# NVIDIA/tensorrt-laboratory

Measured on NVIDIA H100. Metric: ResNet-50 fp16 b=8 inferences/sec, higher is better.
Workload: dtype f16

## Files before the change

### tensorrt_laboratory_b200/csrc/engine.cu

```cuda
#include <cuda.h>
#include <cuda_runtime.h>
#include <stdarg.h>
#include <stdio.h>
#include <stdlib.h>
#include <string.h>

#include <algorithm>
#include <map>
#include <memory>
#include <mutex>
#include <string>
#include <vector>

#include "../../include/b200infer.h"
#include "kernels.h"
#include "plan_format.h"

#include "b2_internal.h"

namespace b2i {
thread_local std::string g_err;
int fail(int code, const char* fmt, ...) {
    char buf[1024];
    va_list ap;
// ... 620 lines not shown
        if (t.last_use < t.def) t.last_use = t.def;
        const size_t size = align_up(t.item_bytes * e->max_batch, 1024);
        const int slack = e->half() ? env_int("B2_ARENA_SLACK", env_int("B2_NET", 0) ? 2 : 0) : 0;
        live.erase(std::remove_if(live.begin(), live.end(), [&](const Live& l) { return l.last + slack < t.def; }), live.end());
        std::sort(live.begin(), live.end(), [](const Live& a, const Live& b) { return a.off < b.off; });
        size_t off = 0;
        for (const Live& l : live) {
            if (off + size <= l.off) break;
            off = std::max(off, l.off + l.size);
        }
        t.offset = off;
        live.push_back({off, size, t.last_use});
        top = std::max(top, off + size);
    }
    e->act_bytes = align_up(std::max<size_t>(top, 1024), 1024);
    e->arena_bytes = e->act_bytes + (e->half() ? kSplitWorkspaceBytes : 0);
}

int make_map_2d(CUtensorMap* map, const void* base, uint64_t inner, uint64_t outer, uint32_t box_inner,
                uint32_t box_outer, CUtensorMapSwizzle swz, bool int8 = false) {
    cuuint64_t dims[2] = {inner, outer};
    cuuint64_t strides[1] = {inner * (int8 ? 1u : 2u)};
    cuuint32_t box[2] = {box_inner, box_outer};
    cuuint32_t estr[2] = {1, 1};
    CUresult r = g_encode_tiled(map, int8 ? CU_TENSOR_MAP_DATA_TYPE_UINT8 : CU_TENSOR_MAP_DATA_TYPE_FLOAT16, 2, const_cast<void*>(base), dims, strides, box,
                                estr, CU_TENSOR_MAP_INTERLEAVE_NONE, swz, CU_TENSOR_MAP_L2_PROMOTION_L2_256B,
                                CU_TENSOR_MAP_FLOAT_OOB_FILL_NONE);
    if (r != CUDA_SUCCESS)
        return fail(B2_ECUDA, "cuTensorMapEncodeTiled failed (%d) dims=%llu,%llu box=%u,%u", int(r),
                    (unsigned long long)inner, (unsigned long long)outer, box_inner, box_outer);
    return B2_OK;
}

int make_map_nhwc(CUtensorMap* map, const void* base, int C, int W, int H, int N, uint32_t box_w, uint32_t box_h) {
    cuuint64_t dims[4] = {cuuint64_t(C), cuuint64_t(W), cuuint64_t(H), cuuint64_t(N)};
    cuuint64_t strides[3] = {cuuint64_t(C) * 2, cuuint64_t(C) * 2 * W, cuuint64_t(C) * 2 * W * H};
    cuuint32_t box[4] = {64, box_w, box_h, 1};
    cuuint32_t estr[4] = {1, 1, 1, 1};
    CUresult r = g_encode_tiled(map, CU_TENSOR_MAP_DATA_TYPE_FLOAT16, 4, const_cast<void*>(base), dims, strides, box, estr,
                                CU_TENSOR_MAP_INTERLEAVE_NONE, CU_TENSOR_MAP_SWIZZLE_128B, CU_TENSOR_MAP_L2_PROMOTION_L2_256B,
                                CU_TENSOR_MAP_FLOAT_OOB_FILL_NONE);
    if (r != CUDA_SUCCESS)
        return fail(B2_ECUDA, "cuTensorMapEncodeTiled(4-D) failed (%d) C=%d W=%d H=%d N=%d box=%u,%u", int(r), C, W, H, N, box_w, box_h);
    return B2_OK;
}

int make_map_im2col(CUtensorMap* map, const void* base, int C, int W, int H, int N, uint64_t pix_bytes,
                    uint64_t row_bytes, uint64_t img_bytes, int kh, int kw, int stride_h, int stride_w, int pad_h,
                    int pad_w_lo, int pad_w_hi, uint32_t channels_per_pixel, uint32_t pixels_per_column,
                    CUtensorMapSwizzle swz, bool int8 = false) {
    cuuint64_t dims[4] = {cuuint64_t(C), cuuint64_t(W), cuuint64_t(H), cuuint64_t(N)};
    cuuint64_t strides[3] = {pix_bytes, row_bytes, img_bytes};
    int lower[2] = {-pad_w_lo, -pad_h};
    int upper[2] = {pad_w_hi - (kw - 1), pad_h - (kh - 1)};
    cuuint32_t estr[4] = {1, cuuint32_t(stride_w), cuuint32_t(stride_h), 1};
    CUresult r = g_encode_im2col(map, int8 ? CU_TENSOR_MAP_DATA_TYPE_UINT8 : CU_TENSOR_MAP_DATA_TYPE_FLOAT16, 4, const_cast<void*>(base), dims, strides, lower,
                                 upper, channels_per_pixel, pixels_per_column, estr, CU_TENSOR_MAP_INTERLEAVE_NONE, swz,
                                 CU_TENSOR_MAP_L2_PROMOTION_L2_256B, CU_TENSOR_MAP_FLOAT_OOB_FILL_NONE);
    if (r != CUDA_SUCCESS)
        return fail(B2_ECUDA, "cuTensorMapEncodeIm2col failed (%d) C=%d W=%d H=%d N=%d k=%dx%d s=%dx%d p=%d,%d/%d", int(r), C,
                    W, H, N, kh, kw, stride_h, stride_w, pad_h, pad_w_lo, pad_w_hi);
    if (g_driver_version <= 13010 && img_bytes * uint64_t(N) < 131072)
        reinterpret_cast<uint64_t*>(map)[1] &= ~(1ull << 21);
    return B2_OK;
}

static int g_sms = 132;

ConvConfig pick_conv_config(int M, int cout_phys, int kblocks, int kb, bool residual, const b2_context* c, bool honor_forced,
                            int group_span = 0) {
    const int m_tiles = (M + 127) / 128;
    ConvConfig best{0, 0, 1, 1e30};
    const int bns[4] = {256, 128, 64, 32};
// ... 8 lines not shown
                               size_t(tiles) * splits * 128 * bn * 4 > kSplitWorkspaceBytes))
                continue;
            const int kpc = (kblocks + splits - 1) / splits;
            if (splits > 1 && (splits - 1) * kpc >= kblocks) continue;
            for (int st : stgs) {
                if (!b2k::conv_config_exists(bn, kb, st)) continue;
                if (b2k::conv_smem_bytes(bn, st, residual) > kSmemLimit) continue;
                if (honor_forced && c->force_stages && st != c->force_stages) continue;
                if (!(honor_forced && c->force_stages) && !stage_depth_useful(bn, kb, st, kpc)) continue;
                const double smem = b2k::conv_smem_bytes(bn, st, residual);
                int per_sm = int(double(kSmemLimit) / smem);
                per_sm = std::min(per_sm, bn <= 64 ? 2 : 1);
                per_sm = std::max(1, std::min(per_sm, 8));
                const int ctas = tiles * splits;
                const int waves = (ctas + g_sms * per_sm - 1) / (g_sms * per_sm);
                const int sharing = std::max(1, std::min(per_sm, (ctas + g_sms - 1) / g_sms));
                const double stage_bytes = 16384.0 + bn * 128.0;
                const double t_kb = std::max(stage_bytes / (70000.0 / sharing), 1.0 / st);
                double t_epi = 0.6 + bn / 64.0 * 0.4 + (residual ? 0.4 : 0.0);
                if (splits > 1) t_epi += 1.0 + 0.3 * splits;
                const double t_cta = 2.0 + kpc * t_kb + t_epi;
                double total = waves * t_cta;
                const double traffic = double(ctas) * kpc * stage_bytes;
                total = std::max(total, traffic / 5.0e6 + 2.0);
                if (total < best.est_us) best = ConvConfig{bn, st, splits, total};
            }
        }
    }
    return best;
}

bool conv_is_row_folded(const b2_context* c, const Op& op) {
    const b2plan::OpRec& r = op.r;
    return !c->no_fold && r.cin_phys == 8 && op.kw() * 8 * 2 == 64 && op.sw() == 1 && op.pw_lo() == 0 && op.pw_hi() == 0;
}
int conv_kb(const b2_context* c, const Op& op) {
    if (op.r.cin_phys % 64 == 0) return 64;
    return conv_is_row_folded(c, op) ? 32 : 8;
}
int conv_num_kblocks(const b2_context* c, const Op& op) {
    const b2plan::OpRec& r = op.r;
    if (op.group_span()) return int(r.taps) * (op.group_span() / 64);
    if (r.cin_phys % 64 == 0) return int(r.taps) * (int(r.cin_phys) / 64);
    if (conv_is_row_folded(c, op)) return (op.kh() + 1) / 2;
    return (int(r.taps_phys) + 7) / 8;
}

int conv_halo_rows(const b2_context* c, const Op& op) {
    const b2plan::OpRec& r = op.r;
    const Tensor& ti = c->e->tensors[r.in];
    const Tensor& to = c->e->tensors[r.out];
    if (op.groups > 1 || r.cin_phys % 64 || r.cout_phys % 64 || op.kh() != 3 || op.kw() != 3 || op.sh() != 1 || op.sw() != 1 || op.ph() != 1 ||
        op.pw_lo() != 1 || op.pw_hi() != 1 || r.res >= 0 || !(r.relu & 2) || ti.h != to.h || ti.w != to.w)
        return 0;
    const int wp = int(to.w) + 2;
    if (wp > 128) return 0;
    return std::min(128 / wp, int(to.h));
}

bool conv_on_tensor_cores(const b2_engine* e, const Op& op) {
    const b2plan::OpRec& r = op.r;
    const bool kb64 = r.cin_phys % 64 == 0, kb8 = r.cin_phys == 8;
    return e->half() && (kb64 || kb8) && r.cout_phys % 32 == 0 && (kb64 || r.taps_phys % 2 == 0) && (op.groups == 1 || op.group_span() > 0);
}

bool conv_takes_ws(const b2_context* c, const Op& op) {
    return conv_kb(c, op) == 64 && (op.r.relu & 2) && op.groups == 1 && !(op.r.relu & b2plan::kConvGelu);
}

bool tactic_applies(const b2_context* c, const Op& op, int batch, const ConvConfig& cfg) {
    const b2plan::OpRec& r = op.r;
    const Tensor& to = c->e->tensors[r.out];
    const int span = op.group_span(), kb = conv_kb(c, op);
    if (cfg.bn <= 0 || int(r.cout_phys) % cfg.bn || cfg.splits < 1 || cfg.sps < 1 || cfg.ws < 0) return false;
    if (op.groups > 1 && (!span || span % cfg.bn || cfg.splits > 1)) return false;
    if ((op.groups > 1 || (r.relu & b2plan::kConvGelu)) && (cfg.ws || cfg.cn > 1 || cfg.halo)) return false;
    if (cfg.halo) {
        const int R = conv_halo_rows(c, op), cblocks = int(r.cin_phys) / 64;
        return R && cfg.splits == 1 && !cfg.ws && cfg.cn <= 1 && b2k::conv_halo_config_exists(cfg.bn) && cblocks <= 8 &&
               b2k::conv_halo_smem(cfg.bn, int(to.w), R, cblocks) <= kSmemLimit;
    }
    if (cfg.ws)
        return conv_takes_ws(c, op) && cfg.splits == 1 && cfg.cn <= 1 && b2k::conv_ws_config_exists(cfg.bn, cfg.stages, cfg.sps) &&
               b2k::conv_ws_smem(cfg.bn, cfg.stages, cfg.sps, r.res >= 0) <= kSmemLimit;
    if (!b2k::conv_config_exists(cfg.bn, kb, cfg.stages, cfg.sps) || b2k::conv_smem_bytes(cfg.bn, cfg.stages, r.res >= 0, cfg.sps) > kSmemLimit)
        return false;
    const int grid_n = int(r.cout_phys) / cfg.bn;
    if (cfg.cn > 1 && (kb != 64 || grid_n % cfg.cn || !b2k::conv_cluster_config_exists(cfg.bn, cfg.stages, cfg.sps, cfg.cn))) return false;
    if (cfg.splits > 1) {
        const int nkb = conv_num_kblocks(c, op), kpc = (nkb + cfg.splits - 1) / cfg.splits;
        const int tiles = (batch * int(to.h * to.w) + 127) / 128 * grid_n;
        if (kb != 64 || kpc < 4 || (cfg.splits - 1) * kpc >= nkb || tiles > kMaxSplitTiles ||
            size_t(tiles) * cfg.splits * 128 * cfg.bn * 4 > kSplitWorkspaceBytes)
            return false;
    }
    return true;
}

std::vector<ConvConfig> conv_candidates(const b2_context* c, const Op& op, int batch, int fixed_splits) {
    const b2plan::OpRec& r = op.r;
    const int kbsz = conv_kb(c, op), nkb = conv_num_kblocks(c, op);
    const int m_tiles = (batch * int(c->e->tensors[r.out].h * c->e->tensors[r.out].w) + 127) / 128;
    const bool ws_only = c->force_ws > 0 && conv_takes_ws(c, op);
    auto ok = [&](const ConvConfig& t) { return tactic_applies(c, op, batch, t); };
    std::vector<ConvConfig> out;
    for (int bn : {256, 128, 64, 32}) {
        if (int(r.cout_phys) % bn) continue;
        const int tiles = m_tiles * (int(r.cout_phys) / bn);
        for (int ws = 0; ws <= 1; ++ws)
        for (int sp : {1, 2, 4, 8})
        for (int sps = 1; sps <= 2; ++sps)
        for (int st : {1, 2, 4, 8}) {
            if ((fixed_splits > 0 && sp != fixed_splits) || (ws ? c->force_ws < 0 : ws_only)) continue;
            ConvConfig t{bn, st, sp, 0.0, sps, ws ? std::min(tiles, g_sms) : 0, 1};
            if (!ok(t)) continue;
            if (ws) {
                if (sps == 2 && nkb < 4) continue;
// ... 80 lines not shown
    a.residual = r.res >= 0 ? reinterpret_cast<const __half*>(tptr(r.res)) : nullptr;
    a.out = reinterpret_cast<__half*>(tptr(r.out));
    a.M = M;
    a.Cout = int(r.cout_phys);
    a.taps = fold ? op.kh() : int(r.taps);
    a.taps_phys = fold ? op.kh() : int(r.taps_phys);
    a.kw = fold ? 1 : op.kw();
    a.cblocks = span ? span / 64 : kb64 ? int(r.cin_phys) / 64 : 1;
    a.group_span = span;
    a.num_kblocks = nkb;
    a.HoWo = int(to.h * to.w);
    a.Wo = int(to.w);
    a.stride_h = op.sh();
    a.stride_w = op.sw();
    a.pad_h = op.ph();
    a.pad_w = op.pw_lo();
    a.relu = int(r.relu & (b2plan::kConvRelu | b2plan::kConvGelu));
    a.wpacked = (r.relu & 2) ? w : nullptr;
    const bool tiled = r.k == 1 && op.kw() == 1 && r.stride == 1 && op.sw() == 1 && r.pad_ == 0 && op.pw_lo() == 0 &&
                       op.pw_hi() == 0 && kb64 && (!c->force_im2col || gelu);
    a.a_mode = tiled ? b2k::A_TILED : b2k::A_IM2COL;
    if (cfg.halo) {
        const int R = conv_halo_rows(c, op);
        cl.halo = 1;
        cl.ws_ctas = 0, cl.cn = 1, a.cn = 1, a.splits = 1, cl.stages = kHaloStagesTag, cl.sps = 1;
        a.halo_rows = R;
        cl.grid_m = batch * ((int(to.h) + R - 1) / R);
        int rc = make_map_nhwc(&cl.mapA, tptr(r.in), int(r.cin_phys), int(ti.w), int(ti.h), batch, uint32_t(ti.w) + 2, uint32_t(R) + 2);
        if (rc) return rc;
        rc = make_map_nhwc(&cl.mapOut, tptr(r.out), int(r.cout_phys), int(to.w), int(to.h), batch, uint32_t(to.w) + 2, uint32_t(R));
        cl.mapB = cl.mapA, cl.mapRes = cl.mapOut;
        return rc;
    }
    const CUtensorMapSwizzle swz = kb64 ? CU_TENSOR_MAP_SWIZZLE_128B : (fold ? CU_TENSOR_MAP_SWIZZLE_64B : CU_TENSOR_MAP_SWIZZLE_NONE);
    const uint64_t pix = uint64_t(r.cin_phys) * 2, rowb = uint64_t(ti.w) * pix, imgb = uint64_t(ti.h) * rowb;
    int rc;
    if (tiled)
        rc = make_map_2d(&cl.mapA, tptr(r.in), r.cin_phys, uint64_t(M), 64, uint32_t(128 / cl.cn), swz);
    else if (fold)
        rc = make_map_im2col(&cl.mapA, tptr(r.in), int(r.cin_phys) * op.kw(), int(ti.w) - op.kw() + 1, int(ti.h), batch, pix,
                             rowb, imgb, op.kh(), 1, op.sh(), 1, op.ph(), 0, 0, 32, 128, swz);
    else
        rc = make_map_im2col(&cl.mapA, tptr(r.in), int(r.cin_phys), int(ti.w), int(ti.h), batch, pix, rowb, imgb, op.kh(),
                             op.kw(), op.sh(), op.sw(), op.ph(), op.pw_lo(), op.pw_hi(), uint32_t(cl.kb), uint32_t(128 / cl.cn), swz);
    if (rc) return rc;
    if (r.relu & 2)
        cl.mapB = cl.mapA;
    else
        rc = make_map_2d(&cl.mapB, w, uint64_t(r.taps_phys) * r.cin_phys, r.cout_phys, uint32_t(cl.kb), uint32_t(cl.bn), swz);
    if (rc) return rc;
    const uint32_t ow = cl.bn >= 64 ? 64 : 32;
    const CUtensorMapSwizzle oswz = cl.bn >= 64 ? CU_TENSOR_MAP_SWIZZLE_128B : CU_TENSOR_MAP_SWIZZLE_64B;
    rc = make_map_2d(&cl.mapOut, tptr(r.out), r.cout_phys, uint64_t(M), ow, 128, oswz);
    if (rc) return rc;
    if (r.res >= 0) rc = make_map_2d(&cl.mapRes, tptr(r.res), r.cout_phys, uint64_t(M), ow, 128, oswz);
    else cl.mapRes = cl.mapOut;
    return rc;
}

int make_i8_conv_launch(b2_context* c, const Op& op, int batch, int bn, int stages, b2k::I8ConvLaunch* out) {
    b2_engine* e = c->e;
    const b2plan::OpRec& r = op.r;
    const Tensor& ti = e->tensors[r.in];
    const Tensor& to = e->tensors[r.out];
    auto tptr = [&](int idx) -> uint8_t* { return c->scratch + e->tensors[idx].offset; };
    b2k::I8ConvLaunch& cl = *out;
    memset(&cl, 0, sizeof cl);
    const int M = batch * int(to.h) * int(to.w);
    cl.bn = bn, cl.stages = stages;
    cl.grid_m = (M + 127) / 128;
    cl.grid_n = int(r.cout_phys) / bn;
    b2k::I8ConvArgs& a = cl.args;
    a.wpacked = e->d_payload + r.w_off;
    const float* rq = reinterpret_cast<const float*>(e->d_payload + r.b_off);
// ... 1465 lines not shown
        if (L.kind == L_NET) run = L.net.get();
    if (!run) return fail(B2_EINVAL, "the plan has no persistent network kernel");
    if (n_ctas) *n_ctas = run->ctas;
    if (run->ctas > cap_ctas) return fail(B2_EINVAL, "counter buffer too small (%d CTAs)", run->ctas);
    long long* d = nullptr;
    const size_t bytes = size_t(run->ctas) * 64 * sizeof(long long);
    B2_CUDA(cudaMalloc(&d, bytes));
    cudaMemset(d, 0, bytes);
    cudaStream_t s = static_cast<cudaStream_t>(stream_);
    run->args.dbg = d;
    int rc = run_all(c, *plan, bindings, s);
    cudaError_t se = cudaStreamSynchronize(s);
    run->args.dbg = nullptr;
    if (!rc && se == cudaSuccess) cudaMemcpy(out, d, bytes, cudaMemcpyDeviceToHost);
    cudaFree(d);
    if (rc) return rc;
    if (se != cudaSuccess) return fail(B2_ECUDA, "debug launch failed: %s", cudaGetErrorString(se));
    return B2_OK;
}

const char* b2_context_launch_name(b2_context* c, int batch, int i) {
    static thread_local std::string s;
    const Launch* L = get_launch(c, batch, i);
    if (!L) return nullptr;
    static const char* kinds[] = {"input_cast", "conv_tcgen05", "conv_simt", "maxpool", "avgpool", "fc", "softmax", "output_cast", "net_tcgen05", "tail_pool_fc_softmax",
                                  "quantize", "conv_i8_tcgen05", "avgpool_i8", "output_cast_i8", "embed_ln", "layernorm", "attention_f16_wgmma",
                                  "pooler", "output_cast_rows"};
    s = std::string(kinds[L->kind]) + ":" + L->name;
    if (L->kind == L_CONV_TC)
        s += " bn=" + std::to_string(L->conv.bn) + " kb=" + std::to_string(L->conv.kb) +
             " st=" + std::to_string(L->conv.stages) + "x" + std::to_string(L->conv.sps) +
             (L->conv.ws_ctas ? " ws=" + std::to_string(L->conv.ws_ctas) : std::string()) +
             (L->conv.cn > 1 ? " cn=" + std::to_string(L->conv.cn) : std::string()) + (L->conv.halo ? " halo" : "") +
             (L->conv.args.a_mode == b2k::A_TILED ? " tiled" : " im2col") +
             " grid=" + std::to_string(L->conv.grid_n) + "x" + std::to_string(L->conv.grid_m) + "x" +
             std::to_string(L->conv.args.splits) + " kblk=" + std::to_string(L->conv.args.num_kblocks) +
             (L->conv.args.group_span ? " span=" + std::to_string(L->conv.args.group_span) : std::string()) +
             ((L->conv.args.relu & b2plan::kConvGelu) ? " gelu" : "");
    if (L->kind == L_CONV_I8)
        s += " bn=" + std::to_string(L->i8.bn) + " st=" + std::to_string(L->i8.stages) + (L->i8.args.a_mode == b2k::A_TILED ? " tiled" : " im2col") + " grid=" +
             std::to_string(L->i8.grid_n) + "x" + std::to_string(L->i8.grid_m) + " kblk=" + std::to_string(L->i8.args.num_kblocks);
    if (L->kind == L_NET)
        s += " layers=" + std::to_string(L->net->args.n_layers) + " tiles=" + std::to_string(L->net->args.total_tiles) +
             " ctas=" + std::to_string(L->net->ctas) + " stages=" + std::to_string(L->net->args.stages);
    if (L->side_join >= 0) s += " side";
    return s.c_str();
}
double b2_context_launch_flops(b2_context* c, int batch, int i) {
    const Launch* L = get_launch(c, batch, i);
    return L ? L->flops : 0.0;
}
double b2_context_launch_bytes(b2_context* c, int batch, int i) {
    const Launch* L = get_launch(c, batch, i);
    return L ? L->bytes : 0.0;
}

}
```

### tensorrt_laboratory_b200/csrc/kernels.cu

```cuda
#include "kernels.h"

#include <stdio.h>
#include <stdlib.h>
#include <string.h>

#include "ptx_sm90.cuh"
#include "wgmma_sm90.cuh"

namespace b2k {

template <int BN, int STAGES, int SPS = 1>
struct ConvCfg {
    static constexpr int A_SUBBLK = 128 * 64 * 2;
    static constexpr int B_SUBBLK = BN * 64 * 2;
    static constexpr int A_STAGE = SPS * A_SUBBLK;
    static constexpr int B_STAGE = SPS * B_SUBBLK;
    static constexpr int PIPE_BYTES = STAGES * (A_STAGE + B_STAGE);
    static constexpr int TILE_BYTES = 128 * BN * 2;
    static_assert(TILE_BYTES <= PIPE_BYTES, "the output staging tile reuses the pipeline buffers");
};

__host__ __device__ constexpr int conv_smem_layout_bytes(int bn, int stages, bool residual, int sps = 1) {
    return stages * sps * (128 * 64 * 2 + bn * 64 * 2) + (residual ? 128 * bn * 2 : 0) + 256 + bn * 4 + 1024;
}

constexpr int kConvThreads = 384;
constexpr int kConsumerWarps = 8;

struct FragPos {
    int row0, col0;
    __device__ FragPos(int consumer_warp, int lane)
        : row0(64 * (consumer_warp >> 2) + 16 * (consumer_warp & 3) + (lane >> 2)), col0(2 * (lane & 3)) {}
};

template <int BN, int KB, int STAGES, int SPS, int CN = 1, bool DBG = false, int AV = 0, bool GELU = false>
__global__ void __launch_bounds__(kConvThreads, BN <= 64 ? 2 : 1)
conv_f16_tcgen05(const __grid_constant__ CUtensorMap mapA, const __grid_constant__ CUtensorMap mapB,
                 const __grid_constant__ CUtensorMap mapOut, const __grid_constant__ CUtensorMap mapRes,
                 const ConvArgs p) {
    static_assert(SPS == 1 || KB == 64, "multi-sub-block stages exist for the 64-wide K path only");
    using Cfg = ConvCfg<BN, STAGES, SPS>;
    constexpr int TPS = 64 / KB;
    constexpr int A_SUB = 128 * KB * 2;
    constexpr int B_SUB = BN * KB * 2;
    constexpr int OW = BN >= 64 ? 64 : 32;
    constexpr int OROWB = OW * 2;
    constexpr int NBOX = BN / OW;

    extern __shared__ uint8_t smem_raw[];
    uint8_t* smem = smem_raw + ((1024u - (smem_u32(smem_raw) & 1023u)) & 1023u);
    const bool has_res = p.residual != nullptr;
    uint8_t* sA = smem;
    uint8_t* sB = smem + STAGES * Cfg::A_STAGE;
    uint8_t* sOut = smem;
    uint8_t* sRes = smem + Cfg::PIPE_BYTES;
    uint8_t* tail = sRes + (has_res ? Cfg::TILE_BYTES : 0);
    uint64_t* full_bar = reinterpret_cast<uint64_t*>(tail);
    uint64_t* empty_bar = full_bar + STAGES;
    uint64_t* accum_bar = empty_bar + STAGES;
    uint64_t* res_bar = accum_bar + 1;
    uint32_t* last_flag = reinterpret_cast<uint32_t*>(res_bar + 1);
    float* s_bias = reinterpret_cast<float*>(tail + 256);

    const int warp = threadIdx.x >> 5;
    const int lane = threadIdx.x & 31;
    const int n0 = blockIdx.x * BN;
    const int m0 = blockIdx.y * 128;
    long long* dbg = (DBG && p.dbg) ? p.dbg + 16ll * ((blockIdx.z * gridDim.y + blockIdx.y) * gridDim.x + blockIdx.x) : nullptr;
    if (dbg && threadIdx.x == 0) {
        dbg[0] = clock64();
        unsigned long long gt;
        asm volatile("mov.u64 %0, %%globaltimer;" : "=l"(gt));
        dbg[8] = static_cast<long long>(gt);
        unsigned smid;
// ... 183 lines not shown
    float acc[BN / 2];
    if (warp >= 4) {
        const uint32_t wg = static_cast<uint32_t>(cw >> 2);
        auto release_stage = [&](int st) {
            __syncwarp();
            if (lane == 0) {
                if (cn > 1) {
                    for (uint32_t r = 0; r < static_cast<uint32_t>(cn); ++r) mbar_arrive_cluster(&empty_bar[st], r);
                } else {
                    mbar_arrive(&empty_bar[st]);
                }
            }
        };
        long long mw = 0, mi = 0;
        for (int i = 0; i < nk; ++i) {
            const int s = i % STAGES;
            const uint32_t ph = (i / STAGES) & 1;
            long long m0c = 0, m1c = 0;
            if (dbg) m0c = clock64();
            mbar_wait(&full_bar[s], ph);
            if (dbg) m1c = clock64(), mw += m1c - m0c;
            if (dbg && i == 0 && cw == 0 && lane == 0) dbg[3] = clock64();
            const uint32_t a_addr = smem_u32(sA + s * Cfg::A_STAGE);
            const uint32_t b_addr = smem_u32(sB + s * Cfg::B_STAGE);
            if constexpr (KB == 64) {
                auto mma = [&](int t) {
                    const int u = t >> 2, j = t & 3;
                    const uint64_t ad = make_wgmma_desc(a_addr + u * Cfg::A_SUBBLK + wg * 8192 + j * 32, 16, 1024, WG_SW128);
                    const uint64_t bd = make_wgmma_desc(b_addr + u * Cfg::B_SUBBLK + j * 32, 16, 1024, WG_SW128);
                    wgmma_f16<BN>(acc, ad, bd, (i > 0 || t > 0) ? 1u : 0u);
                };
                if (SPS == 1 || subs_in_step(i) == SPS) wgmma_group<4 * SPS>(mma);
                else wgmma_group<4>(mma);
            } else if constexpr (KB == 32) {
                auto mma = [&](int t) {
                    const int st = t >> 1, j = t & 1;
                    const uint64_t ad = make_wgmma_desc(a_addr + st * A_SUB + wg * 4096 + j * 32, 16, 512, WG_SW64);
                    const uint64_t bd = make_wgmma_desc(b_addr + st * B_SUB + j * 32, 16, 512, WG_SW64);
                    wgmma_f16<BN>(acc, ad, bd, (i > 0 || t > 0) ? 1u : 0u);
                };
                if (sub_tiles(kb_begin + i) == TPS) wgmma_group<2 * TPS>(mma);
                else wgmma_group<2>(mma);
            } else {
                auto mma = [&](int j) {
                    const uint64_t ad = make_wgmma_desc(a_addr + 2 * j * A_SUB + wg * 1024, A_SUB, 128, WG_NOSWZ);
                    const uint64_t bd = make_wgmma_desc(b_addr + 2 * j * B_SUB, B_SUB, 128, WG_NOSWZ);
                    wgmma_f16<BN>(acc, ad, bd, (i > 0 || j > 0) ? 1u : 0u);
                };
                wgmma_group_upto<TPS / 2>(sub_tiles(kb_begin + i) / 2, mma);
            }
            if constexpr (STAGES == 1) {
                wgmma_wait<0>();
                release_stage(0);
            } else {
                wgmma_wait<1>();
                if (i > 0) release_stage((i - 1) % STAGES);
            }
            if (dbg) mi += clock64() - m1c;
        }
        if constexpr (STAGES > 1) {
            wgmma_wait<0>();
            if (nk > 0) release_stage((nk - 1) % STAGES);
        }
        if (dbg && cw == 0 && lane == 0) dbg[4] = clock64(), dbg[14] = mw, dbg[15] = mi;
    }

    if (warp == 3 && KB == 64) {
        for (int i = 0; i < nk; ++i) {
            const int s = i % STAGES;
            if (i >= STAGES) mbar_wait(&empty_bar[s], ((i / STAGES) & 1) ^ 1);
            if (elect_one_sync()) load_b(kb_begin + i * SPS, s);
            __syncwarp();
        }
    }

// ... 70 lines not shown
                    for (int sp = 0; sp < p.splits; ++sp) {
                        const float2 t = __ldcg(reinterpret_cast<const float2*>(ws_tile + static_cast<size_t>(sp) * (128 * BN) + row * BN + col));
                        f0 += t.x;
                        f1 += t.y;
                    }
                    finish_pair(row, col, f0, f1);
                }
            }
        }
    }
    if (dbg && threadIdx.x == 128) dbg[6] = clock64();
    if (p.pdl_trigger == 2) pdl_launch_dependents();
    fence_proxy_async();
    __syncthreads();
    if (threadIdx.x == 0 && do_store) {
#pragma unroll
        for (int b = 0; b < NBOX; ++b) tma_store_2d(&mapOut, sOut + b * (128 * OROWB), n0 + b * OW, m0);
        tma_store_commit_and_wait_read();
    }
    if (cn > 1) {
        if (warp == 1) {
            const int first = nk > STAGES ? nk - STAGES : 0;
            for (int i = first; i < nk; ++i) mbar_wait(&empty_bar[i % STAGES], (i / STAGES) & 1);
        }
        __syncthreads();
        cluster_sync_all();
    }
    if (dbg && threadIdx.x == 128) {
        dbg[7] = clock64();
        unsigned long long gt;
        asm volatile("mov.u64 %0, %%globaltimer;" : "=l"(gt));
        dbg[9] = static_cast<long long>(gt);
    }
}

__host__ __device__ constexpr int conv_ws_smem_bytes(int bn, int stages, int sps, bool residual) {
    return stages * sps * (128 * 64 * 2 + bn * 64 * 2) + 2 * 128 * bn * 2 + (residual ? 2 * 128 * bn * 2 : 0) + 256 + 1024;
}

template <int BN, int STAGES, int SPS>
__global__ void __launch_bounds__(kConvThreads, 1)
conv_f16_tcgen05_ws(const __grid_constant__ CUtensorMap mapA, const __grid_constant__ CUtensorMap mapOut,
                    const __grid_constant__ CUtensorMap mapRes, const ConvArgs p) {
    constexpr int A_SUBBLK = 128 * 64 * 2;
    constexpr int B_SUBBLK = BN * 64 * 2;
    constexpr int A_STAGE = SPS * A_SUBBLK;
    constexpr int B_STAGE = SPS * B_SUBBLK;
    constexpr int PIPE_BYTES = STAGES * (A_STAGE + B_STAGE);
    constexpr int TILE_BYTES = 128 * BN * 2;
    constexpr int OW = BN >= 64 ? 64 : 32;
    constexpr int OROWB = OW * 2;
    constexpr int NBOX = BN / OW;

    extern __shared__ uint8_t smem_raw[];
    uint8_t* smem = smem_raw + ((1024u - (smem_u32(smem_raw) & 1023u)) & 1023u);
    const bool has_res = p.residual != nullptr;
    uint8_t* sA = smem;
    uint8_t* sB = smem + STAGES * A_STAGE;
    uint8_t* sOut = smem + PIPE_BYTES;
    uint8_t* sRes = sOut + 2 * TILE_BYTES;
    uint8_t* tail = sRes + (has_res ? 2 * TILE_BYTES : 0);
    uint64_t* full_bar = reinterpret_cast<uint64_t*>(tail);
    uint64_t* empty_bar = full_bar + STAGES;
    uint64_t* res_full = empty_bar + STAGES;
    uint64_t* res_empty = res_full + 2;

// ... 402 lines not shown
        }
    }
    return launch_kernel_cluster(conv_f16_tcgen05<BN, KB, STAGES, SPS, CN>, grid, dim3(kConvThreads), smem, stream, true,
                                 static_cast<unsigned>(CN), L.mapA, L.mapB, L.mapOut, L.mapRes, L.args);
}

template <int BN, int KB, int STAGES, int SPS, int CN = 1>
static int init_one() {
    const int want = conv_smem_layout_bytes(BN, STAGES, true, SPS);
    const int bytes = want > 227 * 1024 ? conv_smem_layout_bytes(BN, STAGES, false, SPS) : want;
    if (CN == 1) {
        int e = static_cast<int>(cudaFuncSetAttribute(conv_f16_tcgen05<BN, KB, STAGES, SPS, 1, true>,
                                                      cudaFuncAttributeMaxDynamicSharedMemorySize, bytes));
        if (e) return e;
        if constexpr (KB == 64) {
            if ((e = static_cast<int>(cudaFuncSetAttribute(conv_f16_tcgen05<BN, KB, STAGES, SPS, 1, false, 1>,
                                                           cudaFuncAttributeMaxDynamicSharedMemorySize, bytes)))) return e;
            if ((e = static_cast<int>(cudaFuncSetAttribute(conv_f16_tcgen05<BN, KB, STAGES, SPS, 1, false, 2>,
                                                           cudaFuncAttributeMaxDynamicSharedMemorySize, bytes)))) return e;
            if ((e = static_cast<int>(cudaFuncSetAttribute(conv_f16_tcgen05<BN, KB, STAGES, SPS, 1, false, 2, true>,
                                                           cudaFuncAttributeMaxDynamicSharedMemorySize, bytes)))) return e;
        }
    }
    return static_cast<int>(cudaFuncSetAttribute(conv_f16_tcgen05<BN, KB, STAGES, SPS, CN>, cudaFuncAttributeMaxDynamicSharedMemorySize, bytes));
}

int conv_smem_bytes(int bn, int stages, bool residual, int sps) { return conv_smem_layout_bytes(bn, stages, residual, sps); }

#define B2_FOR_EACH_CONV(X) \
    X(32, 64, 1, 1) X(32, 64, 2, 1) X(32, 64, 4, 1) X(32, 64, 8, 1) \
    X(64, 64, 1, 1) X(64, 64, 2, 1) X(64, 64, 4, 1) X(64, 64, 8, 1) \
    X(128, 64, 1, 1) X(128, 64, 2, 1) X(128, 64, 4, 1) X(256, 64, 2, 1) X(256, 64, 4, 1) \
    X(32, 64, 2, 2) X(32, 64, 4, 2) X(64, 64, 2, 2) X(64, 64, 4, 2) X(128, 64, 2, 2) X(256, 64, 2, 2) \
    X(32, 8, 2, 1) X(32, 8, 4, 1) X(64, 8, 2, 1) X(64, 8, 4, 1) X(64, 8, 8, 1) X(128, 8, 4, 1) \
    X(32, 32, 2, 1) X(32, 32, 4, 1) X(64, 32, 1, 1) X(64, 32, 2, 1) X(64, 32, 4, 1) X(128, 32, 2, 1) X(128, 32, 4, 1)

int conv_halo_smem(int bn, int w, int r, int cblocks) { return halo_smem_bytes(bn, w, r, cblocks); }
bool conv_halo_config_exists(int bn) { return bn == 64 || bn == 128 || bn == 256; }
static int init_conv_halo_kernels() {
    int e;
    if ((e = static_cast<int>(cudaFuncSetAttribute(conv3x3_halo_tcgen05<64>, cudaFuncAttributeMaxDynamicSharedMemorySize, 227 * 1024)))) return e;
    if ((e = static_cast<int>(cudaFuncSetAttribute(conv3x3_halo_tcgen05<128>, cudaFuncAttributeMaxDynamicSharedMemorySize, 227 * 1024)))) return e;
    if ((e = static_cast<int>(cudaFuncSetAttribute(conv3x3_halo_tcgen05<256>, cudaFuncAttributeMaxDynamicSharedMemorySize, 227 * 1024)))) return e;
    return 0;
}
static int launch_conv_halo(const ConvLaunch& L, cudaStream_t stream) {
    const int R = L.args.halo_rows;
    const size_t smem = size_t(halo_smem_bytes(L.bn, L.args.Wo, R, L.args.cblocks));
    if (smem > 227 * 1024 || R < 1 || R * (L.args.Wo + 2) > 128 || L.args.cblocks > kHaloMaxCBlocks) return static_cast<int>(cudaErrorInvalidValue);
    dim3 grid(L.grid_n, L.grid_m, 1);
    switch (L.bn) {
        case 64: return launch_kernel(conv3x3_halo_tcgen05<64>, grid, dim3(kConvThreads), smem, stream, true, L.mapA, L.mapOut, L.args);
        case 128: return launch_kernel(conv3x3_halo_tcgen05<128>, grid, dim3(kConvThreads), smem, stream, true, L.mapA, L.mapOut, L.args);
        case 256: return launch_kernel(conv3x3_halo_tcgen05<256>, grid, dim3(kConvThreads), smem, stream, true, L.mapA, L.mapOut, L.args);
    }
    return static_cast<int>(cudaErrorInvalidValue);
}

#define B2_FOR_EACH_CONV_CLUSTER(X) \
    X(32, 4, 1, 2) X(32, 4, 1, 4) X(64, 1, 1, 2) X(64, 2, 1, 2) X(64, 2, 1, 4) X(64, 2, 2, 2) X(64, 4, 2, 2) X(64, 4, 2, 4) \
    X(128, 2, 1, 2) X(128, 2, 1, 4) X(128, 2, 2, 2)

int init_conv_ws_kernels();
int launch_conv_f16_tcgen05_ws(const ConvLaunch& L, cudaStream_t stream);

int init_conv_kernels() {
    int e = init_conv_ws_kernels();
    if (e) return e;
    if ((e = init_conv_halo_kernels())) return e;
#define B2_INIT(BN_, KB_, ST_, SPS_) \
    if ((e = init_one<BN_, KB_, ST_, SPS_>())) return e;
    B2_FOR_EACH_CONV(B2_INIT)
#undef B2_INIT
#define B2_INIT_CL(BN_, ST_, SPS_, CN_) \
    if ((e = init_one<BN_, 64, ST_, SPS_, CN_>())) return e;
    B2_FOR_EACH_CONV_CLUSTER(B2_INIT_CL)
#undef B2_INIT_CL
    return 0;
}

int launch_conv_f16_tcgen05(const ConvLaunch& L, cudaStream_t stream) {
    if (L.halo) return launch_conv_halo(L, stream);
    if (L.ws_ctas > 0) return launch_conv_f16_tcgen05_ws(L, stream);
    if (L.cn > 1) {
#define B2_CASE_CL(BN_, ST_, SPS_, CN_) \
    if (L.bn == BN_ && L.kb == 64 && L.stages == ST_ && L.sps == SPS_ && L.cn == CN_) return launch_one<BN_, 64, ST_, SPS_, CN_>(L, stream);
        B2_FOR_EACH_CONV_CLUSTER(B2_CASE_CL)
#undef B2_CASE_CL
        return static_cast<int>(cudaErrorInvalidValue);
    }
#define B2_CASE(BN_, KB_, ST_, SPS_) \
    if (L.bn == BN_ && L.kb == KB_ && L.stages == ST_ && L.sps == SPS_) return launch_one<BN_, KB_, ST_, SPS_>(L, stream);
    B2_FOR_EACH_CONV(B2_CASE)
#undef B2_CASE
    return static_cast<int>(cudaErrorInvalidValue);
}

#define B2_FOR_EACH_CONV_WS(X) \
    X(32, 4, 1) X(64, 2, 1) X(64, 4, 1) X(64, 2, 2) X(64, 4, 2) X(128, 2, 1) X(128, 4, 1) X(128, 2, 2)

template <int BN, int STAGES, int SPS>
static int launch_one_ws(const ConvLaunch& L, cudaStream_t stream) {
    const size_t smem = size_t(conv_ws_smem_bytes(BN, STAGES, SPS, L.args.residual != nullptr));
    return launch_kernel(conv_f16_tcgen05_ws<BN, STAGES, SPS>, dim3(L.ws_ctas), dim3(kConvThreads), smem, stream, true, L.mapA, L.mapOut,
                         L.mapRes, L.args);
}

int init_conv_ws_kernels() {
    int e = 0;
#define B2_INIT_WS(BN_, ST_, SPS_)                                                                                        \
    {                                                                                                                     \
        const int want = conv_ws_smem_bytes(BN_, ST_, SPS_, true);                                                        \
        e = static_cast<int>(cudaFuncSetAttribute(conv_f16_tcgen05_ws<BN_, ST_, SPS_>,                                    \
                                                  cudaFuncAttributeMaxDynamicSharedMemorySize,                            \
                                                  want > 227 * 1024 ? conv_ws_smem_bytes(BN_, ST_, SPS_, false) : want)); \
// ... 1 lines not shown
    }
    B2_FOR_EACH_CONV_WS(B2_INIT_WS)
#undef B2_INIT_WS
    return 0;
}

int launch_conv_f16_tcgen05_ws(const ConvLaunch& L, cudaStream_t stream) {
#define B2_CASE_WS(BN_, ST_, SPS_) \
    if (L.bn == BN_ && L.stages == ST_ && L.sps == SPS_) return launch_one_ws<BN_, ST_, SPS_>(L, stream);
    B2_FOR_EACH_CONV_WS(B2_CASE_WS)
#undef B2_CASE_WS
    return static_cast<int>(cudaErrorInvalidValue);
}

bool conv_ws_config_exists(int bn, int stages, int sps) {
#define B2_HAS_WS(BN_, ST_, SPS_) \
    if (bn == BN_ && stages == ST_ && sps == SPS_) return true;
    B2_FOR_EACH_CONV_WS(B2_HAS_WS)
#undef B2_HAS_WS
    return false;
}

int conv_ws_smem(int bn, int stages, int sps, bool residual) { return conv_ws_smem_bytes(bn, stages, sps, residual); }

bool conv_cluster_config_exists(int bn, int stages, int sps, int cn) {
#define B2_HAS_CL(BN_, ST_, SPS_, CN_) \
    if (bn == BN_ && stages == ST_ && sps == SPS_ && cn == CN_) return true;
    B2_FOR_EACH_CONV_CLUSTER(B2_HAS_CL)
#undef B2_HAS_CL
    return false;
}

bool conv_config_exists(int bn, int kb, int stages, int sps) {
#define B2_HAS(BN_, KB_, ST_, SPS_) \
    if (bn == BN_ && kb == KB_ && stages == ST_ && sps == SPS_) return true;
    B2_FOR_EACH_CONV(B2_HAS)
#undef B2_HAS
    return false;
}

static thread_local int B2_LAUNCH_RC = 0;

template <typename T>
struct Acc;
template <>
struct Acc<float> {
    using type = double;
};
template <>
struct Acc<__half> {
    using type = float;
};
__device__ __forceinline__ float to_f(float v) { return v; }
__device__ __forceinline__ float to_f(__half v) { return __half2float(v); }
template <typename T>
__device__ __forceinline__ T from_f(float v);
template <>
__device__ __forceinline__ float from_f<float>(float v) { return v; }
template <>
__device__ __forceinline__ __half from_f<__half>(float v) { return __float2half_rn(v); }

template <typename T>
__global__ void conv_simt_kernel(SimtConvArgs a) {
    pdl_launch_dependents();
    pdl_wait();
    using acc_t = typename Acc<T>::type;
// ... 766 lines not shown
```

### tensorrt_laboratory_b200/csrc/kernels.h

```cpp
#pragma once
#include <cuda.h>
#include <cuda_fp16.h>
#include <cuda_runtime.h>
#include <stdint.h>

namespace b2k {

enum { A_TILED = 0, A_IM2COL = 1 };

struct ConvArgs {
    const float* bias;
    const __half* residual;
    __half* out;
    int M;
    int Cout;
    int num_kblocks;
    int cblocks;
    int taps;
    int taps_phys;
    int kw;
    int HoWo, Wo;
    int stride_h, stride_w;
    int pad_h, pad_w;
    int relu;
    int a_mode;
    int splits;
    int kb_per_split;
    float* workspace;
    int* tile_counters;
    int pdl_trigger;
    const uint8_t* wpacked;
    int halo_rows;
    int cn;
    int tiles_m, tiles_n;
    int dbg_mode;
    long long* dbg;
    int group_span;
};

struct ConvLaunch {
    CUtensorMap mapA;
    CUtensorMap mapB;
    CUtensorMap mapOut;
    CUtensorMap mapRes;
    ConvArgs args;
    int bn;
    int kb;
    int stages;
    int sps;
    int grid_m, grid_n;
    int cn;
    int halo;
    int ws_ctas;
};

int launch_conv_f16_tcgen05(const ConvLaunch& L, cudaStream_t stream);
int init_conv_kernels();
bool conv_config_exists(int bn, int kb, int stages, int sps = 1);
int conv_smem_bytes(int bn, int stages, bool residual, int sps = 1);
bool conv_cluster_config_exists(int bn, int stages, int sps, int cn);
bool conv_halo_config_exists(int bn);
int conv_halo_smem(int bn, int w, int r, int cblocks);
bool conv_ws_config_exists(int bn, int stages, int sps);
int conv_ws_smem(int bn, int stages, int sps, bool residual);
void set_pdl(bool on);
bool get_pdl();

constexpr int kNetMaxLayers = 160;

struct NetLayerInfo {
    const uint8_t* wpacked;
    const float* bias;
    __half* out;
    const __half* residual;
    int M, Cout, num_kblocks, cblocks;
    int kw, HoWo, Wo, stride_h;
    int stride_w, pad_h, pad_w, relu;
    int a_mode, bn, tiles_m, tiles_n;
    int tile_begin, total_tiles;
    int in_flag_off;
    int in_need;
    int res_flag_off, res_need;
    int out_flag_off;
    int dep_off;
    int war_upto;
    int pad_[3];
};
static_assert(sizeof(NetLayerInfo) % 16 == 0, "NetLayerInfo is copied to shared memory in 16-byte words");
struct alignas(64) NetLayer {
    CUtensorMap mapA;
    NetLayerInfo info;
// ... 112 lines not shown
```

Baseline: 30150.

## Add dedicated row-streaming stem conv kernel with resident weights and input row ring

Replaces the im2col-based KB=32 row-folded stem path with a new kernel that keeps all filter rows resident in shared memory, streams input rows through a TMA ring buffer, and reuses each loaded row across the kh output rows that need it. Output rows are written via double-buffered TMA stores, and the grid is split into image/segment/band units sized to the SM count. This targets redundant input reloads in the ResNet-50 7x7 stride-2 stem, at the cost of a new specialised kernel restricted to non-residual, ReLU-only convolutions.

```diff
diff --git a/tensorrt_laboratory_b200/csrc/engine.cu b/tensorrt_laboratory_b200/csrc/engine.cu
--- a/tensorrt_laboratory_b200/csrc/engine.cu
+++ b/tensorrt_laboratory_b200/csrc/engine.cu
@@ -676,13 +676,14 @@
     return B2_OK;
 }
 
-int make_map_nhwc(CUtensorMap* map, const void* base, int C, int W, int H, int N, uint32_t box_w, uint32_t box_h) {
+int make_map_nhwc(CUtensorMap* map, const void* base, int C, int W, int H, int N, uint32_t box_w, uint32_t box_h, uint32_t box_c = 64,
+                  CUtensorMapSwizzle swz = CU_TENSOR_MAP_SWIZZLE_128B) {
     cuuint64_t dims[4] = {cuuint64_t(C), cuuint64_t(W), cuuint64_t(H), cuuint64_t(N)};
     cuuint64_t strides[3] = {cuuint64_t(C) * 2, cuuint64_t(C) * 2 * W, cuuint64_t(C) * 2 * W * H};
-    cuuint32_t box[4] = {64, box_w, box_h, 1};
+    cuuint32_t box[4] = {box_c, box_w, box_h, 1};
     cuuint32_t estr[4] = {1, 1, 1, 1};
     CUresult r = g_encode_tiled(map, CU_TENSOR_MAP_DATA_TYPE_FLOAT16, 4, const_cast<void*>(base), dims, strides, box, estr,
-                                CU_TENSOR_MAP_INTERLEAVE_NONE, CU_TENSOR_MAP_SWIZZLE_128B, CU_TENSOR_MAP_L2_PROMOTION_L2_256B,
+                                CU_TENSOR_MAP_INTERLEAVE_NONE, swz, CU_TENSOR_MAP_L2_PROMOTION_L2_256B,
                                 CU_TENSOR_MAP_FLOAT_OOB_FILL_NONE);
     if (r != CUDA_SUCCESS)
         return fail(B2_ECUDA, "cuTensorMapEncodeTiled(4-D) failed (%d) C=%d W=%d H=%d N=%d box=%u,%u", int(r), C, W, H, N, box_w, box_h);
@@ -757,7 +758,8 @@
 
 bool conv_is_row_folded(const b2_context* c, const Op& op) {
     const b2plan::OpRec& r = op.r;
-    return !c->no_fold && r.cin_phys == 8 && op.kw() * 8 * 2 == 64 && op.sw() == 1 && op.pw_lo() == 0 && op.pw_hi() == 0;
+    return !c->no_fold && r.cin_phys == 8 && op.kw() * 8 * 2 == 64 && op.sw() == 1 && op.pw_lo() == 0 && op.pw_hi() == 0 &&
+           r.res < 0 && !(r.relu & (2 | b2plan::kConvGelu)) && b2k::conv_stem_smem(64, op.kh(), op.sh()) > 0;
 }
 int conv_kb(const b2_context* c, const Op& op) {
     if (op.r.cin_phys % 64 == 0) return 64;
@@ -808,6 +810,10 @@
     if (cfg.ws)
         return conv_takes_ws(c, op) && cfg.splits == 1 && cfg.cn <= 1 && b2k::conv_ws_config_exists(cfg.bn, cfg.stages, cfg.sps) &&
                b2k::conv_ws_smem(cfg.bn, cfg.stages, cfg.sps, r.res >= 0) <= kSmemLimit;
+    if (kb == 32) {
+        const int smem = b2k::conv_stem_smem(cfg.bn, op.kh(), op.sh());
+        return b2k::conv_config_exists(cfg.bn, kb, cfg.stages, cfg.sps) && cfg.splits == 1 && cfg.cn <= 1 && smem > 0 && smem <= kSmemLimit;
+    }
     if (!b2k::conv_config_exists(cfg.bn, kb, cfg.stages, cfg.sps) || b2k::conv_smem_bytes(cfg.bn, cfg.stages, r.res >= 0, cfg.sps) > kSmemLimit)
         return false;
     const int grid_n = int(r.cout_phys) / cfg.bn;
@@ -954,14 +960,28 @@
         cl.mapB = cl.mapA, cl.mapRes = cl.mapOut;
         return rc;
     }
-    const CUtensorMapSwizzle swz = kb64 ? CU_TENSOR_MAP_SWIZZLE_128B : (fold ? CU_TENSOR_MAP_SWIZZLE_64B : CU_TENSOR_MAP_SWIZZLE_NONE);
+    if (fold) {
+        const int Ho = int(to.h), Wo = int(to.w);
+        a.stem_segs = (Wo + 127) / 128;
+        const int units = std::max(1, 2 * g_sms / cl.grid_n);
+        const int bands = std::min(Ho, std::max(1, units / (batch * a.stem_segs)));
+        a.stem_band_rows = (Ho + bands - 1) / bands;
+        a.stem_bands = (Ho + a.stem_band_rows - 1) / a.stem_band_rows;
+        cl.grid_m = batch * a.stem_segs * a.stem_bands;
+        int rc = make_map_nhwc(&cl.mapA, tptr(r.in), 8, int(ti.w), int(ti.h), batch, b2k::kStemBoxPix, 1, 8, CU_TENSOR_MAP_SWIZZLE_NONE);
+        if (!rc)
+            rc = make_map_2d(&cl.mapB, w, uint64_t(r.taps_phys) * r.cin_phys, r.cout_phys, 32, uint32_t(cl.bn), CU_TENSOR_MAP_SWIZZLE_64B);
+        if (!rc)
+            rc = make_map_nhwc(&cl.mapOut, tptr(r.out), int(r.cout_phys), Wo, Ho, batch, 128, 1, cl.bn >= 64 ? 64 : 32,
+                               cl.bn >= 64 ? CU_TENSOR_MAP_SWIZZLE_128B : CU_TENSOR_MAP_SWIZZLE_64B);
+        cl.mapRes = cl.mapOut;
+        return rc;
+    }
+    const CUtensorMapSwizzle swz = kb64 ? CU_TENSOR_MAP_SWIZZLE_128B : CU_TENSOR_MAP_SWIZZLE_NONE;
     const uint64_t pix = uint64_t(r.cin_phys) * 2, rowb = uint64_t(ti.w) * pix, imgb = uint64_t(ti.h) * rowb;
     int rc;
     if (tiled)
         rc = make_map_2d(&cl.mapA, tptr(r.in), r.cin_phys, uint64_t(M), 64, uint32_t(128 / cl.cn), swz);
-    else if (fold)
-        rc = make_map_im2col(&cl.mapA, tptr(r.in), int(r.cin_phys) * op.kw(), int(ti.w) - op.kw() + 1, int(ti.h), batch, pix,
-                             rowb, imgb, op.kh(), 1, op.sh(), 1, op.ph(), 0, 0, 32, 128, swz);
     else
         rc = make_map_im2col(&cl.mapA, tptr(r.in), int(r.cin_phys), int(ti.w), int(ti.h), batch, pix, rowb, imgb, op.kh(),
                              op.kw(), op.sh(), op.sw(), op.ph(), op.pw_lo(), op.pw_hi(), uint32_t(cl.kb), uint32_t(128 / cl.cn), swz);
@@ -2493,7 +2513,7 @@
              " st=" + std::to_string(L->conv.stages) + "x" + std::to_string(L->conv.sps) +
              (L->conv.ws_ctas ? " ws=" + std::to_string(L->conv.ws_ctas) : std::string()) +
              (L->conv.cn > 1 ? " cn=" + std::to_string(L->conv.cn) : std::string()) + (L->conv.halo ? " halo" : "") +
-             (L->conv.args.a_mode == b2k::A_TILED ? " tiled" : " im2col") +
+             (L->conv.kb == 32 ? " rows" : L->conv.args.a_mode == b2k::A_TILED ? " tiled" : " im2col") +
              " grid=" + std::to_string(L->conv.grid_n) + "x" + std::to_string(L->conv.grid_m) + "x" +
              std::to_string(L->conv.args.splits) + " kblk=" + std::to_string(L->conv.args.num_kblocks) +
              (L->conv.args.group_span ? " span=" + std::to_string(L->conv.args.group_span) : std::string()) +
diff --git a/tensorrt_laboratory_b200/csrc/kernels.cu b/tensorrt_laboratory_b200/csrc/kernels.cu
--- a/tensorrt_laboratory_b200/csrc/kernels.cu
+++ b/tensorrt_laboratory_b200/csrc/kernels.cu
@@ -40,6 +40,7 @@
                  const ConvArgs p) {
     static_assert(SPS == 1 || KB == 64, "multi-sub-block stages exist for the 64-wide K path only");
     using Cfg = ConvCfg<BN, STAGES, SPS>;
+    static_assert(KB == 64 || KB == 8, "the row-folded stem (KB = 32) has its own kernel, conv_stem_rows");
     constexpr int TPS = 64 / KB;
     constexpr int A_SUB = 128 * KB * 2;
     constexpr int B_SUB = BN * KB * 2;
@@ -289,15 +290,6 @@
                 };
                 if (SPS == 1 || subs_in_step(i) == SPS) wgmma_group<4 * SPS>(mma);
                 else wgmma_group<4>(mma);
-            } else if constexpr (KB == 32) {
-                auto mma = [&](int t) {
-                    const int st = t >> 1, j = t & 1;
-                    const uint64_t ad = make_wgmma_desc(a_addr + st * A_SUB + wg * 4096 + j * 32, 16, 512, WG_SW64);
-                    const uint64_t bd = make_wgmma_desc(b_addr + st * B_SUB + j * 32, 16, 512, WG_SW64);
-                    wgmma_f16<BN>(acc, ad, bd, (i > 0 || t > 0) ? 1u : 0u);
-                };
-                if (sub_tiles(kb_begin + i) == TPS) wgmma_group<2 * TPS>(mma);
-                else wgmma_group<2>(mma);
             } else {
                 auto mma = [&](int j) {
                     const uint64_t ad = make_wgmma_desc(a_addr + 2 * j * A_SUB + wg * 1024, A_SUB, 128, WG_NOSWZ);
@@ -434,6 +426,147 @@
         asm volatile("mov.u64 %0, %%globaltimer;" : "=l"(gt));
         dbg[9] = static_cast<long long>(gt);
     }
+}
+
+constexpr int kStemSlotTx = kStemBoxPix * 16;
+constexpr int kStemSlotBytes = (kStemSlotTx + 127) / 128 * 128;
+__host__ __device__ constexpr int stem_ring_slots(int kh, int sh) { return kh + 2 * sh; }
+__host__ __device__ constexpr int stem_smem_layout_bytes(int bn, int kh, int sh) {
+    return kh * bn * 64 + 2 * 128 * bn * 2 + stem_ring_slots(kh, sh) * kStemSlotBytes + 256 + bn * 4 + 1024;
+}
+constexpr int kStemMaxKh = 8, kStemMaxSh = 2;
+
+template <int BN>
+__global__ void __launch_bounds__(kConvThreads, BN <= 64 ? 2 : 1)
+conv_stem_rows(const __grid_constant__ CUtensorMap mapIn, const __grid_constant__ CUtensorMap mapB,
+               const __grid_constant__ CUtensorMap mapOut, const ConvArgs p) {
+    constexpr int OW = BN >= 64 ? 64 : 32;
+    constexpr int OROWB = OW * 2;
+    constexpr int NBOX = BN / OW;
+    constexpr int W_ROW = BN * 64;
+    constexpr int OUT_TILE = 128 * BN * 2;
+
+    extern __shared__ uint8_t smem_raw[];
+    uint8_t* smem = smem_raw + ((1024u - (smem_u32(smem_raw) & 1023u)) & 1023u);
+    const int kh = p.taps, sh = p.stride_h, ns = stem_ring_slots(kh, sh);
+    uint8_t* sW = smem;
+    uint8_t* sOut = sW + kh * W_ROW;
+    uint8_t* sRing = sOut + 2 * OUT_TILE;
+    uint64_t* w_bar = reinterpret_cast<uint64_t*>(sRing + ns * kStemSlotBytes);
+    uint64_t* full_bar = w_bar + 1;
+    uint64_t* empty_bar = full_bar + ns;
+    float* s_bias = reinterpret_cast<float*>(reinterpret_cast<uint8_t*>(w_bar) + 256);
+
+    const int warp = threadIdx.x >> 5;
+    const int lane = threadIdx.x & 31;
+    const int n0 = blockIdx.x * BN;
+    const int Ho = p.HoWo / p.Wo;
+    const int per_img = p.stem_segs * p.stem_bands;
+    const int img = blockIdx.y / per_img;
+    const int seg = (blockIdx.y - img * per_img) / p.stem_bands;
+    const int band = blockIdx.y - img * per_img - seg * p.stem_bands;
+    const int p0 = band * p.stem_band_rows;
+    const int nrows = min(Ho - p0, p.stem_band_rows);
+    const int q0 = seg * 128;
+    const int h0 = p0 * sh - p.pad_h;
+    const int n_in = (nrows - 1) * sh + kh;
+
+    if (threadIdx.x == 0) {
+        tma_prefetch_desc(&mapIn);
+        tma_prefetch_desc(&mapB);
+        tma_prefetch_desc(&mapOut);
+        mbar_init(w_bar, 1);
+        for (int s = 0; s < ns; ++s) {
+            mbar_init(&full_bar[s], 1);
+            mbar_init(&empty_bar[s], static_cast<uint32_t>(kConsumerWarps));
+        }
+        fence_barrier_init();
+        fence_proxy_async();
+    }
+    if (warp == 3) {
+#pragma unroll
+        for (int i = 0; i < BN / 32; ++i) s_bias[lane + 32 * i] = __ldg(p.bias + n0 + lane + 32 * i);
+    }
+    __syncthreads();
+    if (p.pdl_trigger == 0) pdl_launch_dependents();
+
+    if (warp == 0) {
+        if (elect_one_sync()) {
+            mbar_expect_tx(w_bar, static_cast<uint32_t>(kh * W_ROW));
+            for (int r = 0; r < kh; ++r) tma_load_2d(&mapB, w_bar, sW + r * W_ROW, r * 32, n0);
+        }
+        __syncwarp();
+        pdl_wait();
+        int s = 0;
+        uint32_t ph = 0;
+        for (int i = 0; i < n_in; ++i) {
+            if (i >= ns) mbar_wait(&empty_bar[s], ph ^ 1);
+            if (elect_one_sync()) {
+                mbar_expect_tx(&full_bar[s], kStemSlotTx);
+                tma_load_4d(&mapIn, &full_bar[s], sRing + s * kStemSlotBytes, 0, q0, h0 + i, img);
+            }
+            __syncwarp();
+            if (++s == ns) s = 0, ph ^= 1;
+        }
+    } else if (warp >= 4) {
+        const int cw = warp - 4;
+        const uint32_t wg = static_cast<uint32_t>(cw >> 2);
+        const FragPos fp(cw, lane);
+        const bool issuer = threadIdx.x == 128;
+        const uint32_t w_addr = smem_u32(sW);
+        const uint32_t a_base = smem_u32(sRing) + wg * (64 * 16);
+        pdl_wait();
+        mbar_wait(w_bar, 0);
+        float acc[BN / 2];
+        int s0 = 0;
+        for (int pl = 0; pl < nrows; ++pl) {
+            const int i0 = pl * sh;
+            for (int r = 0, s = s0; r < kh; ++r, s = s + 1 == ns ? 0 : s + 1)
+                mbar_wait(&full_bar[s], static_cast<uint32_t>((i0 + r) / ns) & 1u);
+            auto row_mma = [&](int r) {
+                const int s = s0 + r >= ns ? s0 + r - ns : s0 + r;
+                const uint32_t a_addr = a_base + static_cast<uint32_t>(s * kStemSlotBytes);
+#pragma unroll
+                for (int j = 0; j < 2; ++j) {
+                    const uint64_t ad = make_wgmma_desc(a_addr + j * 32, 16, 128, WG_NOSWZ);
+                    const uint64_t bd = make_wgmma_desc(w_addr + r * W_ROW + j * 32, 16, 512, WG_SW64);
+                    wgmma_f16<BN>(acc, ad, bd, (r > 0 || j > 0) ? 1u : 0u);
+                }
+            };
+            wgmma_group_upto<kStemMaxKh>(kh, row_mma);
+            wgmma_wait<0>();
+            __syncwarp();
+            if (lane == 0)
+                for (int r = 0, s = s0; r < sh; ++r, s = s + 1 == ns ? 0 : s + 1) mbar_arrive(&empty_bar[s]);
+            s0 = s0 + sh >= ns ? s0 + sh - ns : s0 + sh;
+
+            uint8_t* out = sOut + (pl & 1) * OUT_TILE;
+            if (issuer && pl >= 2) tma_store_wait_read1();
+            named_bar_sync(1, 256);
+#pragma unroll
+            for (int j = 0; j < BN / 8; ++j)
+#pragma unroll
+                for (int h = 0; h < 2; ++h) {
+                    const int row = fp.row0 + 8 * h, col = 8 * j + fp.col0;
+                    const uint32_t so = static_cast<uint32_t>((col / OW) * (128 * OROWB)) + swz_off<OROWB>(row, (col % OW) / 8) + (col % 8) * 2;
+                    float v0 = acc[4 * j + 2 * h] + s_bias[col], v1 = acc[4 * j + 2 * h + 1] + s_bias[col + 1];
+                    if (p.relu) {
+                        v0 = fmaxf(v0, 0.0f);
+                        v1 = fmaxf(v1, 0.0f);
+                    }
+                    *reinterpret_cast<__half2*>(out + so) = __floats2half2_rn(v0, v1);
+                }
+            fence_proxy_async();
+            named_bar_sync(1, 256);
+            if (issuer) {
+#pragma unroll
+                for (int b = 0; b < NBOX; ++b) tma_store_4d(&mapOut, out + b * (128 * OROWB), n0 + b * OW, q0, p0 + pl, img);
+                tma_store_commit();
+            }
+        }
+        if (issuer) tma_store_wait_read0();
+    }
+    if (p.pdl_trigger != 0) pdl_launch_dependents();
 }
 
 __host__ __device__ constexpr int conv_ws_smem_bytes(int bn, int stages, int sps, bool residual) {
@@ -902,8 +1035,35 @@
     X(64, 64, 1, 1) X(64, 64, 2, 1) X(64, 64, 4, 1) X(64, 64, 8, 1) \
     X(128, 64, 1, 1) X(128, 64, 2, 1) X(128, 64, 4, 1) X(256, 64, 2, 1) X(256, 64, 4, 1) \
     X(32, 64, 2, 2) X(32, 64, 4, 2) X(64, 64, 2, 2) X(64, 64, 4, 2) X(128, 64, 2, 2) X(256, 64, 2, 2) \
-    X(32, 8, 2, 1) X(32, 8, 4, 1) X(64, 8, 2, 1) X(64, 8, 4, 1) X(64, 8, 8, 1) X(128, 8, 4, 1) \
-    X(32, 32, 2, 1) X(32, 32, 4, 1) X(64, 32, 1, 1) X(64, 32, 2, 1) X(64, 32, 4, 1) X(128, 32, 2, 1) X(128, 32, 4, 1)
+    X(32, 8, 2, 1) X(32, 8, 4, 1) X(64, 8, 2, 1) X(64, 8, 4, 1) X(64, 8, 8, 1) X(128, 8, 4, 1)
+
+int conv_stem_smem(int bn, int kh, int stride_h) {
+    if ((bn != 32 && bn != 64 && bn != 128) || kh < 1 || kh > kStemMaxKh || stride_h < 1 || stride_h > kStemMaxSh || stride_h > kh)
+        return 0;
+    return stem_smem_layout_bytes(bn, kh, stride_h);
+}
+static int init_conv_stem_kernels() {
+    int e;
+    if ((e = static_cast<int>(cudaFuncSetAttribute(conv_stem_rows<32>, cudaFuncAttributeMaxDynamicSharedMemorySize,
+                                                   stem_smem_layout_bytes(32, kStemMaxKh, kStemMaxSh)))))
+        return e;
+    if ((e = static_cast<int>(cudaFuncSetAttribute(conv_stem_rows<64>, cudaFuncAttributeMaxDynamicSharedMemorySize,
+                                                   stem_smem_layout_bytes(64, kStemMaxKh, kStemMaxSh)))))
+        return e;
+    return static_cast<int>(cudaFuncSetAttribute(conv_stem_rows<128>, cudaFuncAttributeMaxDynamicSharedMemorySize,
+                                                 stem_smem_layout_bytes(128, kStemMaxKh, kStemMaxSh)));
+}
+static int launch_conv_stem(const ConvLaunch& L, cudaStream_t stream) {
+    const size_t smem = size_t(conv_stem_smem(L.bn, L.args.taps, L.args.stride_h));
+    if (smem == 0 || L.args.splits != 1 || L.args.residual != nullptr || (L.args.relu & ~1)) return static_cast<int>(cudaErrorInvalidValue);
+    const dim3 grid(L.grid_n, L.grid_m, 1);
+    switch (L.bn) {
+        case 32: return launch_kernel(conv_stem_rows<32>, grid, dim3(kConvThreads), smem, stream, true, L.mapA, L.mapB, L.mapOut, L.args);
+        case 64: return launch_kernel(conv_stem_rows<64>, grid, dim3(kConvThreads), smem, stream, true, L.mapA, L.mapB, L.mapOut, L.args);
+        case 128: return launch_kernel(conv_stem_rows<128>, grid, dim3(kConvThreads), smem, stream, true, L.mapA, L.mapB, L.mapOut, L.args);
+    }
+    return static_cast<int>(cudaErrorInvalidValue);
+}
 
 int conv_halo_smem(int bn, int w, int r, int cblocks) { return halo_smem_bytes(bn, w, r, cblocks); }
 bool conv_halo_config_exists(int bn) { return bn == 64 || bn == 128 || bn == 256; }
@@ -938,6 +1098,7 @@
     int e = init_conv_ws_kernels();
     if (e) return e;
     if ((e = init_conv_halo_kernels())) return e;
+    if ((e = init_conv_stem_kernels())) return e;
 #define B2_INIT(BN_, KB_, ST_, SPS_) \
     if ((e = init_one<BN_, KB_, ST_, SPS_>())) return e;
     B2_FOR_EACH_CONV(B2_INIT)
@@ -951,6 +1112,7 @@
 
 int launch_conv_f16_tcgen05(const ConvLaunch& L, cudaStream_t stream) {
     if (L.halo) return launch_conv_halo(L, stream);
+    if (L.kb == 32) return launch_conv_stem(L, stream);
     if (L.ws_ctas > 0) return launch_conv_f16_tcgen05_ws(L, stream);
     if (L.cn > 1) {
 #define B2_CASE_CL(BN_, ST_, SPS_, CN_) \
@@ -1018,6 +1180,7 @@
 }
 
 bool conv_config_exists(int bn, int kb, int stages, int sps) {
+    if (kb == 32) return stages == 1 && sps == 1 && (bn == 32 || bn == 64 || bn == 128);
 #define B2_HAS(BN_, KB_, ST_, SPS_) \
     if (bn == BN_ && kb == KB_ && stages == ST_ && sps == SPS_) return true;
     B2_FOR_EACH_CONV(B2_HAS)
diff --git a/tensorrt_laboratory_b200/csrc/kernels.h b/tensorrt_laboratory_b200/csrc/kernels.h
--- a/tensorrt_laboratory_b200/csrc/kernels.h
+++ b/tensorrt_laboratory_b200/csrc/kernels.h
@@ -36,6 +36,9 @@
     int dbg_mode;
     long long* dbg;
     int group_span;
+    int stem_band_rows;
+    int stem_bands;
+    int stem_segs;
 };
 
 struct ConvLaunch {
@@ -54,9 +57,12 @@
     int ws_ctas;
 };
 
+constexpr int kStemBoxPix = 128 + 3;
+
 int launch_conv_f16_tcgen05(const ConvLaunch& L, cudaStream_t stream);
 int init_conv_kernels();
 bool conv_config_exists(int bn, int kb, int stages, int sps = 1);
+int conv_stem_smem(int bn, int kh, int stride_h);
 int conv_smem_bytes(int bn, int stages, bool residual, int sps = 1);
 bool conv_cluster_config_exists(int bn, int stages, int sps, int cn);
 bool conv_halo_config_exists(int bn);
```

After: 30440 (median of 6 runs). About the same (+1.0%).
